# TorontoDeepLearning/convnet

Measured on NVIDIA H100. Metric: images/sec ImageNet AlexNet training, higher is better.
Workload: dtype bf16

## Files before the change

### convnet_b200/csrc/conv_tc.cu

```cuda
#include <cuda.h>
#include <cuda_bf16.h>
#include <cudaTypedefs.h>

#include <algorithm>
#include <vector>

#include "conv_kernels.h"
#include "sm90_ptx.cuh"

namespace cnb {

namespace {

constexpr int kConsumerWarps = 8;
template <int SW> constexpr int kThreadsFor = 32 * (kConsumerWarps + 1 + SW);
constexpr int BM = 128;
constexpr int BN_MAX = 128;
constexpr int BK = 32;
constexpr int kMaxStages = 8;
constexpr uint32_t kAStageBytes = BM * 128;
constexpr uint32_t kBStageBytes = BN_MAX * 128;

enum Op { kFprop = 0, kDgrad = 1, kWgrad = 2 };

struct TcParams {
  int bf16, chunk, chunk_shift, cpt, bk, nbc;
  int N, nb;
  int W, H, modX, modY, modules;
  int Cin, Cout;
  int kx, ky, sx, sy, px, py, taps;
  int frames, frame0;
  int BN, stages;
  int m_tiles, n_tiles, num_tiles;
  int kc_blocks;
  int x_mode, x_yblocks, x_ct;
  const float* xw;
  uint32_t bank_bytes;
  uint32_t epi_bytes;
  uint32_t b_tx_bytes;
  int a_merged, b_merged;
  int untied;
  int total_chunks;
  int splits, units_per_split;
  long long part_stride;
  float* out;
  __nv_bfloat16* out16;
  int vec;
  float st, so;
  const float* bias; int act;
  const float* mask; int mask_act;
  float drop_prob, drop_scale;
  unsigned long long drop_seed;
  long long out_frame_step;
  int o_sx, o_sy, o_x0, o_y0, o_W;
  long long out_plane;
};

struct __align__(8) SmemCtl {
  uint64_t full[kMaxStages];
  uint64_t empty[kMaxStages];
  uint64_t epi_full;
  uint64_t epi_empty;
};

struct Tile {
  int m_tile, n_tile;
  int tap, o_tile, c_tile, split;
};

template <int OP>
// ... 258 lines not shown
        const long long idx = row + col_stride * col;
        const float a[4] = {acc[k].x, acc[k].y, acc[k].z, acc[k].w};
        const float o[4] = {old[k].x, old[k].y, old[k].z, old[k].w};
        const float m[4] = {msk[k].x, msk[k].y, msk[k].z, msk[k].w};
        float v[4];
#pragma unroll
        for (int e = 0; e < 4; e++) {
          float r = so_eff * a[e];
          if (rmw) r += p.st * o[e];
          if (OP == kFprop) {
            if (bias) r += bv[k];
            if (SIG) { if (p.act) r = act_apply(r, p.act); }
            else if (p.act) r = fmaxf(r, 0.f);
            if (p.drop_scale != 0.f) r *= dropout_keep(p.drop_seed + (unsigned long long)(idx + e), p.drop_prob, p.drop_scale);
          }
          if (SIG) { if (p.mask) r = act_deriv(r, m[e], p.mask_act); }
          else if (p.mask && !(m[e] > 0.f)) r = 0.f;
          v[e] = r;
        }
        acc[k] = make_float4(v[0], v[1], v[2], v[3]);
      }
      if ((rmw || p.mask) && b + 1 < batches) load_batch(b + 1);
#pragma unroll
      for (int k = 0; k < kEpiCols; k++) {
        const int col = c0 + kStoreWarps * k;
        if (col >= ncols) continue;
        const long long idx = row + col_stride * col;
        const float v[4] = {acc[k].x, acc[k].y, acc[k].z, acc[k].w};
        float* const dst = p.out + idx;
        if (vec) {
          *reinterpret_cast<float4*>(dst) = acc[k];
        } else {
#pragma unroll
          for (int e = 0; e < 4; e++) dst[e] = v[e];
        }
        if (p.out16) {
          __nv_bfloat16* const d16 = p.out16 + idx;
          const __nv_bfloat162 lo = __floats2bfloat162_rn(v[0], v[1]), hi = __floats2bfloat162_rn(v[2], v[3]);
          if (vec) {
            uint2 w;
            w.x = *reinterpret_cast<const uint32_t*>(&lo);
            w.y = *reinterpret_cast<const uint32_t*>(&hi);
            *reinterpret_cast<uint2*>(d16) = w;
          } else {
            d16[0] = lo.x; d16[1] = lo.y; d16[2] = hi.x; d16[3] = hi.y;
          }
        }
      }
    }
    phase ^= 1;
  }
}

template <int OP, bool BF16, bool SIG, int SW>
__global__ void __launch_bounds__(kThreadsFor<SW>, 1)
tc_conv_kernel(const __grid_constant__ CUtensorMap mapA, const __grid_constant__ CUtensorMap mapB, const __grid_constant__ TcParams p) {
  extern __shared__ uint8_t smem_raw[];
  uint8_t* smem = reinterpret_cast<uint8_t*>((reinterpret_cast<uintptr_t>(smem_raw) + 1023) & ~uintptr_t(1023));
  uint8_t* smemA = smem;
  uint8_t* smemB = smem + (size_t)p.stages * kAStageBytes;
  uint8_t* smemE = smemB + (p.bank_bytes ? (size_t)p.bank_bytes : (size_t)p.stages * kBStageBytes);
  SmemCtl* ctl = reinterpret_cast<SmemCtl*>(smemE + p.epi_bytes);

  const int warp = __shfl_sync(0xffffffffu, (int)(threadIdx.x >> 5), 0), lane = threadIdx.x & 31;

  if (threadIdx.x == 0) {
    for (int s = 0; s < p.stages; s++) { ptx::mbar_init(&ctl->full[s], 1); ptx::mbar_init(&ctl->empty[s], kConsumerWarps); }
    ptx::mbar_init(&ctl->epi_full, kConsumerWarps);
    ptx::mbar_init(&ctl->epi_empty, SW);
    ptx::fence_barrier_init();
    ptx::tma_prefetch_desc(&mapA);
    ptx::tma_prefetch_desc(&mapB);
  }
  __syncthreads();
  ptx::pdl_launch_dependents();
  ptx::pdl_wait();

  if (warp > kConsumerWarps) {
    if constexpr (OP != kWgrad) store_tiles<OP, SIG, SW>(p, ctl, ptx::smem_u32(smemE), warp - kConsumerWarps - 1, lane);
    return;
  }
  if (warp == kConsumerWarps) {
    if (lane != 0) return;
    int stage = 0; uint32_t phase = 0;
    const uint32_t tx_bytes = kAStageBytes + p.b_tx_bytes;
    for (int t = blockIdx.x; t < p.num_tiles; t += gridDim.x) {
      const Tile tile = decode_tile<OP>(p, t);
      auto begin_stage = [&]() -> uint8_t* {
        ptx::mbar_wait(&ctl->empty[stage], phase ^ 1);
        ptx::mbar_arrive_expect_tx(&ctl->full[stage], tx_bytes);
        return smemA + (size_t)stage * kAStageBytes;
      };
      auto lda5 = [&](const void* m, void* dst, int c0, int c1, int c2, int c3, int c4) {
        ptx::tma_load_5d(m, &ctl->full[stage], dst, c0, c1, c2, c3, c4);
      };
      auto lda4 = [&](const void* m, void* dst, int c0, int c1, int c2, int c3) {
        ptx::tma_load_4d(m, &ctl->full[stage], dst, c0, c1, c2, c3);
      };
      auto lda3 = [&](const void* m, void* dst, int c0, int c1, int c2) {
        ptx::tma_load_3d(m, &ctl->full[stage], dst, c0, c1, c2);
      };
      auto end_stage = [&]() { if (++stage == p.stages) { stage = 0; phase ^= 1; } };

      if (OP == kFprop) {
        const Chunks ch = decode_chunks(p, tile.m_tile, p.modules);
        int cX[4], cY[4];
#pragma unroll
        for (int c = 0; c < 4; c++) {
          cX[c] = (ch.pos[c] % p.modX) * p.sx + p.px;
          cY[c] = (ch.pos[c] / p.modX) * p.sy + p.py;
        }
        if (p.x_mode) {
          for (int c = 0; c < p.Cin; c++)
            for (int yb = 0; yb < p.x_yblocks; yb++) {
              uint8_t* a = begin_stage();
              if (p.a_merged) {
                lda5(&mapA, a, 0, cX[0], cY[0] + 4 * yb, ch.n[0] >> 5, c);
              } else {
#pragma unroll
                for (int q = 0; q < 4; q++)
                  lda5(&mapA, a + q * (BK * 128), ch.n[q], c, cX[q], cY[q] + 4 * yb, ch.f[q]);
              }
              end_stage();
            }
        } else {
          const int cb0 = p.splits > 1 ? tile.split * p.units_per_split : 0;
          const int cb1 = p.splits > 1 ? min(cb0 + p.units_per_split, p.kc_blocks) : p.kc_blocks;
          const int mod = ch.pos[0];
          for (int ty = 0; ty < p.ky; ty++)
            for (int tx = 0; tx < p.kx; tx++) {
              const int tap = tx + p.kx * ty;
              for (int cb = cb0; cb < cb1; cb++) {
                uint8_t* a = begin_stage();
                uint8_t* b = smemB + (size_t)stage * kBStageBytes;
                if (p.a_merged) {
                  lda5(&mapA, a, 0, cb * p.bk, ch.n[0] >> p.chunk_shift, cX[0] + tx, cY[0] + ty);
                } else {
#pragma unroll
                  for (int c = 0; c < 4; c++)
                    if (c < p.cpt) lda5(&mapA, a + c * (p.bk * 128), ch.n[c], cb * p.bk, cX[c] + tx, cY[c] + ty, ch.f[c]);
                }
                const int o0 = tile.n_tile * p.BN;
                if (p.b_merged) {
                  if (p.untied) lda5(&mapB, b, 0, cb * p.bk, o0 >> p.chunk_shift, tap, mod);
                  else lda4(&mapB, b, 0, cb * p.bk, o0 >> p.chunk_shift, tap);
                } else {
                  for (int j = 0; j < ((p.BN + p.chunk - 1) >> p.chunk_shift); j++) {
                    if (p.untied) lda4(&mapB, b + j * (p.bk * 128), o0 + j * p.chunk, tap, cb * p.bk, mod);
                    else lda3(&mapB, b + j * (p.bk * 128), o0 + j * p.chunk, tap, cb * p.bk);
                  }
                }
                end_stage();
              }
            }
        }
      } else if (OP == kDgrad) {
        const Chunks ch = decode_chunks(p, tile.m_tile, p.W * p.H);
        const DgradTaps taps = dgrad_taps(p, ch);
        const bool none = dgrad_live_taps(p, taps) == 0;
        int cX[4], cY[4];
#pragma unroll
        for (int c = 0; c < 4; c++) { cX[c] = ch.pos[c] % p.W; cY[c] = ch.pos[c] / p.W; }
        const int ob0 = p.splits > 1 ? tile.split * p.units_per_split : 0;
        const int ob1 = p.splits > 1 ? min(ob0 + p.units_per_split, p.kc_blocks) : p.kc_blocks;
        for (int ty = 0; ty < p.ky; ty++)
          for (int tx = 0; tx < p.kx; tx++) {
            if (!(taps.any(tx, ty) || (none && tx == 0 && ty == 0))) continue;
            int mx[4], my[4];
#pragma unroll
            for (int c = 0; c < 4; c++) {
              const bool lv = ch.ok[c] && taps.live(c, tx, ty);
              mx[c] = lv ? (cX[c] - p.px - tx) / p.sx : -1;
              my[c] = lv ? (cY[c] - p.py - ty) / p.sy : -1;
            }
            const int tap = tx + p.kx * ty;
            const int mod = mx[0] >= 0 ? mx[0] + p.modX * my[0] : -1;
            for (int ob = ob0; ob < ob1; ob++) {
              uint8_t* a = begin_stage();
              uint8_t* b = smemB + (size_t)stage * kBStageBytes;
              if (p.a_merged) {
                lda5(&mapA, a, 0, ob * p.bk, ch.n[0] >> p.chunk_shift, mx[0], my[0]);
              } else {
#pragma unroll
                for (int c = 0; c < 4; c++)
                  if (c < p.cpt) lda5(&mapA, a + c * (p.bk * 128), ch.n[c], ob * p.bk, mx[c], my[c], p.frame0);
              }
              if (p.untied) lda4(&mapB, b, ob * p.bk, tap, tile.n_tile * p.BN, mod);
              else lda3(&mapB, b, ob * p.bk, tap, tile.n_tile * p.BN);
              end_stage();
            }
          }
      } else if (p.untied) {
        const int mx = tile.split % p.modX, my = tile.split / p.modX;
        const int X = mx * p.sx + p.px + tile.tap % p.kx, Y = my * p.sy + p.py + tile.tap / p.kx;
        for (int ib = 0; ib < p.nbc; ib++) {
          uint8_t* a = begin_stage();
          uint8_t* b = smemB + (size_t)stage * kBStageBytes;
          lda5(&mapA, a, ib * p.chunk, mx, my, tile.o_tile * BM, 0);
          lda5(&mapB, b, ib * p.chunk, X, Y, tile.c_tile * p.BN, 0);
          end_stage();
        }
      } else if (p.x_mode) {
        const int r0 = tile.split * p.units_per_split, r1 = min(r0 + p.units_per_split, p.modY * p.frames);
        const uint32_t c_bytes = (uint32_t)p.ky * 8 * 128;
        for (int r = r0; r < r1; r++) {
          const int f = r / p.modY, my = r % p.modY;
          for (int mx = 0; mx < p.modX; mx++)
            for (int ib = 0; ib < p.nb; ib++) {
              uint8_t* a = begin_stage();
              uint8_t* b = smemB + (size_t)stage * kBStageBytes;
              lda5(&mapA, a, ib * 32, mx, my, tile.o_tile * BM, f);
              for (int c = 0; c < p.x_ct; c++)
                lda5(&mapB, b + c * c_bytes, ib * 32, mx * p.sx + p.px, my * p.sy + p.py, tile.c_tile * p.x_ct + c, f);
              end_stage();
            }
        }
      } else {
        const WgradSpan sp = wgrad_span(p, tile);
        const int tx = tile.tap % p.kx, ty = tile.tap / p.kx;
        if (sp.live_rows == 0 || sp.mx_hi < sp.mx_lo) {
          for (int ib = 0; ib < p.nbc; ib++) {
            uint8_t* a = begin_stage();
            uint8_t* b = smemB + (size_t)stage * kBStageBytes;
            lda5(&mapA, a, ib * p.chunk, 0, 0, tile.o_tile * BM, 0);
            lda5(&mapB, b, ib * p.chunk, -1, -1, tile.c_tile * p.BN, 0);
            end_stage();
          }
        } else {
          for (int r = sp.r0; r < sp.r1; r++) {
            if (!wgrad_row_live(p, r, ty)) continue;
            const int f = r / p.modY, my = r % p.modY;
            const int Y = my * p.sy + p.py + ty;
            for (int mx = sp.mx_lo; mx <= sp.mx_hi; mx++) {
              const int X = mx * p.sx + p.px + tx;
              for (int ib = 0; ib < p.nbc; ib++) {
                uint8_t* a = begin_stage();
                uint8_t* b = smemB + (size_t)stage * kBStageBytes;
                lda5(&mapA, a, ib * p.chunk, mx, my, tile.o_tile * BM, f);
                lda5(&mapB, b, ib * p.chunk, X, Y, tile.c_tile * p.BN, f);
                end_stage();
              }
            }
          }
        }
      }
    }
    return;
  }

  const int g = lane >> 2, tq = lane & 3;
  const int row0 = warp * 16 + g;
  int stage = 0; uint32_t phase = 0;
  int bank_tile = -1;
  uint32_t epi_phase = 0;
  for (int t = blockIdx.x; t < p.num_tiles; t += gridDim.x) {
    const Tile tile = decode_tile<OP>(p, t);
    const int nkb = tile_kblocks<OP>(p, tile);
    float acc[BN_MAX / 8][4];
#pragma unroll
    for (int j = 0; j < BN_MAX / 8; j++)
#pragma unroll
      for (int e = 0; e < 4; e++) acc[j][e] = 0.f;

    if constexpr (BF16 || OP == kWgrad) {
      constexpr bool a_mn = (OP != kWgrad), b_mn = (OP == kFprop);
      constexpr uint32_t a_step = a_mn ? 2048u : 32u, b_step = b_mn ? 2048u : 32u;
      const uint64_t da0 = ptx::gmma_desc(ptx::smem_u32(smemA) + (uint32_t)(warp >> 2) * 8192u, a_mn ? 8192u : 16u, 1024u);
      const uint64_t db0 = ptx::gmma_desc(ptx::smem_u32(smemB), b_mn ? 8192u : 16u, 1024u);
      int prev = -1;
      ptx::wgmma_fence_operands(acc);
      for (int kb = 0; kb < nkb; kb++) {
        ptx::mbar_wait(&ctl->full[stage], phase);
        ptx::wgmma_fence();
        const uint64_t da = da0 + ((uint32_t)stage * kAStageBytes >> 4), db = db0 + ((uint32_t)stage * kBStageBytes >> 4);
#pragma unroll
        for (int ks = 0; ks < 4; ks++) {
          if constexpr (BF16)
            ptx::wgmma_m64n128k16_bf16<a_mn ? 1 : 0, b_mn ? 1 : 0>(acc, da + (ks * a_step >> 4), db + (ks * b_step >> 4));
          else
            ptx::wgmma_m64n128k8_tf32(acc, da + (ks * a_step >> 4), db + (ks * b_step >> 4));
        }
        ptx::wgmma_commit();
        ptx::wgmma_wait<1>();
        if (prev >= 0 && lane == 0) ptx::mbar_arrive(&ctl->empty[prev]);
        prev = stage;
        if (++stage == p.stages) { stage = 0; phase ^= 1; }
      }
      ptx::wgmma_wait<0>();
      ptx::wgmma_fence_operands(acc);
      if (prev >= 0 && lane == 0) ptx::mbar_arrive(&ctl->empty[prev]);
    } else if (OP == kFprop && p.x_mode) {
      if (tile.n_tile != bank_tile) {
        ptx::bar_sync(1, 32 * kConsumerWarps);
        xmode_fill_bank(p, smemB, tile.n_tile);
        ptx::fence_proxy_async_smem();
        ptx::bar_sync(1, 32 * kConsumerWarps);
        bank_tile = tile.n_tile;
      }
      const uint32_t sA = ptx::smem_u32(smemA), bank = ptx::smem_u32(smemB);
      switch (p.BN) {
        case 32: xmode_fprop_mma<32>(acc, p, ctl, sA, bank, nkb, stage, phase, row0, tq, lane); break;
        case 64: xmode_fprop_mma<64>(acc, p, ctl, sA, bank, nkb, stage, phase, row0, tq, lane); break;
        case 96: xmode_fprop_mma<96>(acc, p, ctl, sA, bank, nkb, stage, phase, row0, tq, lane); break;
        default: xmode_fprop_mma<128>(acc, p, ctl, sA, bank, nkb, stage, phase, row0, tq, lane); break;
      }
    } else {
      const uint32_t sA = ptx::smem_u32(smemA), sB = ptx::smem_u32(smemB);
      constexpr bool b_mn = (OP == kFprop);
      for (int kb = 0; kb < nkb; kb++) {
        ptx::mbar_wait(&ctl->full[stage], phase);
        const uint32_t A = sA + (uint32_t)stage * kAStageBytes, B = sB + (uint32_t)stage * kBStageBytes;
#pragma unroll
        for (int ks = 0; ks < 4; ks++) {
          const int k0 = ks * 8 + tq, k1 = k0 + 4;
          const uint32_t a0 = ptx::lds32(A + off_mnmajor(row0, k0));
          const uint32_t a1 = ptx::lds32(A + off_mnmajor(row0 + 8, k0));
          const uint32_t a2 = ptx::lds32(A + off_mnmajor(row0, k1));
          const uint32_t a3 = ptx::lds32(A + off_mnmajor(row0 + 8, k1));
#pragma unroll
          for (int j = 0; j < BN_MAX / 8; j++) {
            if (j * 8 >= p.BN) break;
            const int n = j * 8 + g;
            const uint32_t b0 = ptx::lds32(B + (b_mn ? off_mnmajor(n, k0) : off_kmajor(n, k0)));
            const uint32_t b1 = ptx::lds32(B + (b_mn ? off_mnmajor(n, k1) : off_kmajor(n, k1)));
            ptx::mma_tf32_16x8x8(acc[j], a0, a1, a2, a3, b0, b1);
          }
        }
        __syncwarp();
        if (lane == 0) ptx::mbar_arrive(&ctl->empty[stage]);
        if (++stage == p.stages) { stage = 0; phase ^= 1; }
      }
    }

    if constexpr (OP != kWgrad) {
      ptx::mbar_wait(&ctl->epi_empty, epi_phase ^ 1);
      uint32_t base[2][2];
#pragma unroll
      for (int h = 0; h < 2; h++)
#pragma unroll
        for (int e = 0; e < 2; e++) base[h][e] = ptx::smem_u32(smemE) + epi_off(row0 + 8 * h, 2 * tq + e);
#pragma unroll
      for (int j = 0; j < BN_MAX / 8; j++) {
        if (j * 8 >= p.BN) break;
#pragma unroll
        for (int h = 0; h < 2; h++)
#pragma unroll
          for (int e = 0; e < 2; e++) ptx::sts32(base[h][e] + j * 8 * BM * 4, acc[j][2 * h + e]);
      }
      __syncwarp();
      if (lane == 0) ptx::mbar_arrive(&ctl->epi_full);
      epi_phase ^= 1;
    } else {
      float* rowp[2] = {nullptr, nullptr};
      long long col_stride = 0;
#pragma unroll
      for (int h = 0; h < 2; h++) {
        const int o = tile.o_tile * BM + row0 + 8 * h;
        if (o < p.Cout) {
          rowp[h] = p.out + (long long)tile.split * p.Cout * p.taps * p.Cin + o;
          if (!p.x_mode) {
            col_stride = (long long)p.Cout * p.taps;
            rowp[h] += (long long)p.Cout * tile.tap + col_stride * ((long long)tile.c_tile * p.BN);
          }
        }
      }
      const int ncols_valid = p.x_mode ? min(p.BN, p.x_ct * p.ky * 8) : min(p.BN, p.Cin - tile.c_tile * p.BN);
      const bool direct_scale = (p.splits == 1) || p.untied;
      const float so_eff = direct_scale ? p.so : 1.f;
      const bool rmw = direct_scale && p.st != 0.f;
      auto dst_of = [&](float* rp, int col) -> float* {
        if (p.x_mode) {
          const int tx = col & 7, rr = col >> 3, ty = rr % p.ky, c = tile.c_tile * p.x_ct + rr / p.ky;
          if (tx >= p.kx || c >= p.Cin) return nullptr;
          return rp + (long long)p.Cout * (tx + p.kx * (ty + p.ky * c));
        }
        return rp + col_stride * col;
      };
#pragma unroll
      for (int h = 0; h < 2; h++) {
        float* const rp = rowp[h];
        if (rp == nullptr) continue;
#pragma unroll
        for (int j = 0; j < BN_MAX / 8; j++)
#pragma unroll
          for (int e = 0; e < 2; e++) {
            const int col = j * 8 + 2 * tq + e;
            if (col >= ncols_valid) continue;
            float* const dst = dst_of(rp, col);
            if (dst == nullptr) continue;
            float r = so_eff * acc[j][2 * h + e];
            if (rmw) r += p.st * *dst;
            *dst = r;
          }
      }
    }
  }
}

PFN_cuTensorMapEncodeTiled_v12000 encode_fn() {
  static PFN_cuTensorMapEncodeTiled_v12000 fn = nullptr;
  if (!fn) {
    void* ptr = nullptr;
    cudaDriverEntryPointQueryResult qres;
    CNB_CUDA_CHECK(cudaGetDriverEntryPoint("cuTensorMapEncodeTiled", &ptr, cudaEnableDefault, &qres));
    CNB_REQUIRE(qres == cudaDriverEntryPointSuccess && ptr != nullptr, "cuTensorMapEncodeTiled");
    fn = reinterpret_cast<PFN_cuTensorMapEncodeTiled_v12000>(ptr);
  }
  return fn;
}

struct Elem { int bf16, esz, chunk, shift, bk; };
inline Elem elem_for(bool bf16) { return bf16 ? Elem{1, 2, 64, 6, 64} : Elem{0, 4, 32, 5, 32}; }

bool make_map(CUtensorMap* map, const void* base, const Elem& e, int rank, const long long* dims, const long long* strides,
              const int* box) {
  cuuint64_t gdim[5], gstr[4];
  cuuint32_t bdim[5], estr[5];
  if ((reinterpret_cast<uintptr_t>(base) & 15) != 0) return false;
  for (int i = 0; i < rank; i++) {
    if (dims[i] <= 0 || dims[i] > 0xFFFFFFFFLL) return false;
    gdim[i] = (cuuint64_t)dims[i];
    bdim[i] = (cuuint32_t)box[i];
    estr[i] = 1;
    if (box[i] > 256) return false;
    if (i > 0) {
      const long long bytes = strides[i - 1] * e.esz;
      if (bytes % 16 != 0 || bytes <= 0 || bytes >= (1LL << 40)) return false;
      gstr[i - 1] = (cuuint64_t)bytes;
    }
  }
  CUresult r = encode_fn()(map, e.bf16 ? CU_TENSOR_MAP_DATA_TYPE_BFLOAT16 : CU_TENSOR_MAP_DATA_TYPE_FLOAT32, (cuuint32_t)rank,
                           const_cast<void*>(base), gdim, gstr, bdim, estr, CU_TENSOR_MAP_INTERLEAVE_NONE,
                           CU_TENSOR_MAP_SWIZZLE_128B, CU_TENSOR_MAP_L2_PROMOTION_L2_256B, CU_TENSOR_MAP_FLOAT_OOB_FILL_NONE);
  if (r != CUDA_SUCCESS) {
    fprintf(stderr, "convnet_b200: cuTensorMapEncodeTiled failed (%d)\n", (int)r);
    return false;
  }
  return true;
}

int pick_bn(int cols, int granule) {
  const int tiles = ceil_div(cols, BN_MAX);
  const int bn = ceil_div(ceil_div(cols, tiles), granule) * granule;
  return std::min(BN_MAX, std::max(granule, bn));
}

size_t smem_bytes_for(int stages, uint32_t bank_bytes, uint32_t epi_bytes) {
  const size_t b = bank_bytes ? (size_t)bank_bytes : (size_t)stages * kBStageBytes;
  return 1024 + (size_t)stages * kAStageBytes + b + epi_bytes + sizeof(SmemCtl) + 16;
}
constexpr size_t kSmemBudget = 227 * 1024;
inline uint32_t epi_bytes_for(int bn) { return (uint32_t)BM * bn * 4; }

int pick_stages(uint32_t bank_bytes, uint32_t epi_bytes) {
  int s = kMaxStages;
  while (s > 2 && smem_bytes_for(s, bank_bytes, epi_bytes) > kSmemBudget) s--;
  return s;
}

int pick_store_warps(int kblocks, double tile_bytes) {
  const double mma_us = 0.3 * kblocks;
  const double epi_us = tile_bytes / (3e6 / 132);
  return 2.0 * epi_us >= mma_us ? 7 : 3;
}

template <int OP, bool BF16, bool SIG, int SW>
void launch_one(const CUtensorMap& a, const CUtensorMap& b, const TcParams& p, size_t smem) {
  smem_opt_in(tc_conv_kernel<OP, BF16, SIG, SW>, 227 * 1024);
  const int grid = std::min(p.num_tiles, num_sms());
  launch_pdl(tc_conv_kernel<OP, BF16, SIG, SW>, dim3((unsigned)grid), dim3(kThreadsFor<SW>), smem, state().stream, a, b, p);
}

template <int OP>
void launch(const CUtensorMap& a, const CUtensorMap& b, TcParams& p) {
  p.epi_bytes = OP == kWgrad ? 0u : epi_bytes_for(p.BN);
  p.stages = pick_stages(p.bank_bytes, p.epi_bytes);
  const size_t smem = smem_bytes_for(p.stages, p.bank_bytes, p.epi_bytes);
  auto aligned = [](const void* q, uintptr_t a) { return (reinterpret_cast<uintptr_t>(q) & (a - 1)) == 0; };
  p.vec = aligned(p.out, 16) && aligned(p.mask, 16) && aligned(p.out16, 8) ? 1 : 0;
  const bool sig = p.act == kActLogistic || (p.mask && p.mask_act == kActLogistic);
  CNB_REQUIRE(OP != kWgrad || !sig, "tc_conv: wgrad has no activation epilogue");
  void (*run)(const CUtensorMap&, const CUtensorMap&, const TcParams&, size_t) = nullptr;
  if constexpr (OP != kWgrad) {
    const int kcb = p.splits > 1 ? p.units_per_split : p.kc_blocks;
    const int kblocks = (OP == kFprop && p.x_mode) ? p.Cin * p.x_yblocks : p.taps * kcb;
    const double bytes = BM * p.BN * (4.0 + (p.out16 ? 2 : 0) + (p.mask ? 4 : 0) + (p.st != 0.f && p.splits == 1 ? 4 : 0));
    if (pick_store_warps(kblocks, bytes) == 7) {
      if (sig) run = p.bf16 ? launch_one<OP, true, true, 7> : launch_one<OP, false, true, 7>;
      else run = p.bf16 ? launch_one<OP, true, false, 7> : launch_one<OP, false, false, 7>;
    } else if (sig) {
      run = p.bf16 ? launch_one<OP, true, true, 3> : launch_one<OP, false, true, 3>;
    }
  }
  if (!run) run = p.bf16 ? launch_one<OP, true, false, 3> : launch_one<OP, false, false, 3>;
  run(a, b, p, smem);
  count_launch();
  CNB_LAUNCH_CHECK("tc_conv");
}

void fill_common(TcParams& p, const ConvGeom& g, const Elem& e) {
  p.bf16 = e.bf16; p.chunk = e.chunk; p.chunk_shift = e.shift; p.cpt = BM / e.chunk; p.bk = e.bk;
  p.N = g.N; p.nb = ceil_div(g.N, 32); p.nbc = ceil_div(g.N, e.chunk);
  p.W = g.W; p.H = g.H; p.modX = g.modX; p.modY = g.modY; p.modules = g.modules;
  p.Cin = g.Cin; p.Cout = g.Cout;
  p.kx = g.kx; p.ky = g.ky; p.sx = g.sx; p.sy = g.sy; p.px = g.px; p.py = g.py; p.taps = g.kx * g.ky;
  p.frames = g.frames; p.frame0 = 0;
  p.splits = 1; p.units_per_split = 0; p.part_stride = 0;
  p.x_mode = 0; p.x_yblocks = 0; p.x_ct = 0; p.b_tx_bytes = 0;
  p.xw = nullptr; p.bank_bytes = 0; p.epi_bytes = 0;
  p.a_merged = 0; p.b_merged = 0;
  p.untied = g.conv ? 0 : 1;
  p.bias = nullptr; p.act = 0; p.mask = nullptr; p.mask_act = 0; p.out16 = nullptr; p.vec = 0;
  p.drop_prob = 0.f; p.drop_scale = 0.f; p.drop_seed = 0;
  p.o_sx = p.o_sy = 1; p.o_x0 = p.o_y0 = 0; p.o_W = g.modX; p.out_plane = g.modules;
  p.out_frame_step = g.out_frame_step;
  p.total_chunks = 0;
  p.st = 0.f; p.so = 1.f; p.out = nullptr;
}

bool image_map(CUtensorMap* m, const void* base, const Elem& e, const ConvGeom& g, int Wd, int Hd, int C,
               long long frame_step, bool channel_second, int box_c) {
  const long long N = g.N;
  if (channel_second) {
    const long long dims[5] = {N, C, Wd, Hd, g.frames};
    const long long str[4] = {N * Wd * Hd, N, N * Wd, frame_step};
    const int box[5] = {e.chunk, box_c, 1, 1, 1};
    return make_map(m, base, e, 5, dims, str, box);
  }
  const long long dims[5] = {N, Wd, Hd, C, g.frames};
  const long long str[4] = {N, N * Wd, N * Wd * Hd, frame_step};
  const int box[5] = {e.chunk, 1, 1, box_c, 1};
  return make_map(m, base, e, 5, dims, str, box);
}

bool merged_image_map(CUtensorMap* m, const void* base, const Elem& e, const ConvGeom& g, int Wd, int Hd, int C, bool x_mode) {
  const long long N = g.N;
  if (x_mode) {
    const long long dims[5] = {32, Wd, Hd, N / 32, C};
    const long long str[4] = {N, N * Wd, 32, N * Wd * Hd};
    const int box[5] = {32, 8, 4, 4, 1};
    return make_map(m, base, e, 5, dims, str, box);
  }
  const long long dims[5] = {e.chunk, C, N / e.chunk, Wd, Hd};
  const long long str[4] = {N * Wd * Hd, e.chunk, N, N * Wd};
  const int box[5] = {e.chunk, e.bk, BM / e.chunk, 1, 1};
// ... 239 lines not shown
  {
    const long long dims[4] = {g.Cout, (long long)g.kx * g.ky, g.Cin, g.modules};
    const long long str[3] = {g.Cout, (long long)g.Cout * g.kx * g.ky, (long long)g.Cout * g.K};
    const int box[4] = {e.chunk, 1, p.BN, 1};
    if (!make_map(&mb, buf.y, e, g.conv ? 3 : 4, dims, str, box)) return {};
  }
  float* out = targets + (long long)g.cin0 * g.H * g.W * g.N;
  bool emit = false;
  if (whole && p.splits > 1) {
    p.st = 0.f; p.out = buf.part; p.mask = nullptr;
    launch<kDgrad>(ma, mb, p);
    reduce_split(buf.part, out, out_elems, p.splits, st, so, nullptr, 1, 0, fuse.act_state, fuse.state_act);
  } else if (whole) {
    p.st = st; p.out = out; p.mask = fuse.act_state ? fuse.act_state + (long long)g.cin0 * g.H * g.W * g.N : nullptr;
    p.mask_act = fuse.state_act;
    p.out16 = out16;
    emit = out16 != nullptr;
    launch<kDgrad>(ma, mb, p);
  } else {
    scale_buffer(targets, g.img_total, st);
    p.st = 1.f;
    for (int f = 0; f < g.frames; f++) {
      p.frame0 = f; p.out = out + f * g.in_frame_step;
      launch<kDgrad>(ma, mb, p);
    }
  }
  return {bf ? kPathTcBf16 : kPathTcTf32, emit, false};
}
ConvOutcome tc_conv_down(const ConvGeom& g, const float* derivs, const float* filters, float* targets, float st, float so,
                         const Fuse& fuse, __nv_bfloat16* out16) {
  if (want_bf16()) {
    ConvOutcome r;
    if (st == 0.f) r = tc_conv_down_as_fprop(g, derivs, filters, targets, so, fuse, out16);
    if (r.path == kPathNone) r = tc_conv_down_impl(g, derivs, filters, targets, st, so, fuse, out16, true);
    if (r.path != kPathNone) return r;
  }
  return tc_conv_down_impl(g, derivs, filters, targets, st, so, fuse, out16, false);
}

static ConvPath tc_conv_outp_impl(const ConvGeom& g, const float* images, const float* derivs, float* targets, float st,
                                  float so, bool bf) {
  const Elem e = elem_for(bf);
  if (g.N % 4 != 0 || g.Cout < 8) return kPathNone;
  const bool x_mode = g.Cin < 8;
  if (x_mode && (g.kx > 8 || g.ky > 8)) return kPathNone;
  if (bf && (x_mode || g.N % 8 != 0 || !aligned16(images) || !aligned16(derivs))) return kPathNone;
  if (!g.conv && (g.N % 128 != 0 || g.frames != 1 || x_mode)) return kPathNone;
  if (bf && (long long)g.N * g.modules * g.frames < 1024 && !(g.frames == 1 && g.N % 128 == 0 && g.Cin % 32 == 0)) return kPathNone;
  TcParams p; fill_common(p, g, e);
  p.kc_blocks = 0;
  p.m_tiles = ceil_div(g.Cout, BM);
  if (x_mode) {
    p.x_mode = 1;
    p.x_ct = std::min(g.Cin, BN_MAX / (8 * g.ky));
    p.BN = ceil_div(p.x_ct * g.ky * 8, 16) * 16;
    p.n_tiles = ceil_div(g.Cin, p.x_ct);
    p.b_tx_bytes = (uint32_t)p.x_ct * g.ky * 8 * 128;
  } else {
    p.BN = pick_bn(g.Cin, 16);
    p.n_tiles = ceil_div(g.Cin, p.BN);
    p.b_tx_bytes = (uint32_t)p.BN * 128;
  }
  const int units = g.modY * g.frames;
  const long long base_tiles = (long long)(x_mode ? 1 : p.taps) * p.m_tiles * p.n_tiles;
  int splits;
  {
    const long long slots = num_sms();
    const double row_us = 0.3 * g.modX * std::max(1, p.nbc / 2);
    const double dw_bytes = 4.0 * g.Cout * g.K;
    const int cap = (int)std::max<long long>(1, std::min<long long>(units, (4LL * num_sms()) / std::max<long long>(base_tiles, 1)));
    double best = 1e30; splits = 1;
    for (int sp = 1; sp <= cap; sp++) {
      const int ups = ceil_div(units, sp), real = ceil_div(units, ups);
      const long long waves = ceil_div<long long>(base_tiles * real, slots);
      const double cost = (double)waves * (ups * row_us + 1.5) + (real > 1 ? dw_bytes * (real + 1) / 3e6 : 0.0);
      if (cost < best - 1e-9) { best = cost; splits = real; }
    }
  }
  const long long elems = (long long)g.Cout * g.K;
  while (splits > 1 && elems * splits * 4 > (1LL << 30)) splits--;
  p.units_per_split = ceil_div(units, splits);
  p.splits = ceil_div(units, p.units_per_split);
  if (!g.conv) {
    if (base_tiles * g.modules >= (1LL << 31)) return kPathNone;
    p.splits = g.modules; p.units_per_split = 1;
  }
  p.num_tiles = (int)(base_tiles * p.splits);
  p.st = st; p.so = so;
  CUtensorMap ma, mb;
  const bool partials = p.splits > 1 && g.conv;
  const size_t part_bytes = partials ? align_up(sizeof(float) * elems * p.splits) : 0;
  const CallBuffers buf = call_buffers(bf, part_bytes, {images, g.img_total, (long long)g.cin0 * g.H * g.W * g.N},
                                       {derivs, g.out_total, (long long)g.cout0 * g.modules * g.N});
  if (!image_map(&ma, buf.y, e, g, g.modX, g.modY, g.Cout, g.out_frame_step, false, BM)) return kPathNone;
  if (x_mode) {
    const long long N = g.N;
    const long long dims[5] = {N, g.W, g.H, g.Cin, g.frames};
    const long long str[4] = {N, N * g.W, N * g.W * g.H, g.in_frame_step};
    const int box[5] = {32, 8, g.ky, 1, 1};
    if (!make_map(&mb, buf.x, e, 5, dims, str, box)) return kPathNone;
  } else if (!image_map(&mb, buf.x, e, g, g.W, g.H, g.Cin, g.in_frame_step, false, p.BN)) return kPathNone;
  p.out = partials ? buf.part : targets;
  launch<kWgrad>(ma, mb, p);
  if (partials) reduce_partials(buf.part, targets, elems, 1, p.splits, st, so);
  return bf ? kPathTcBf16 : kPathTcTf32;
}
ConvPath tc_conv_outp(const ConvGeom& g, const float* images, const float* derivs, float* targets, float st, float so) {
  if (want_bf16()) {
    const ConvPath path = tc_conv_outp_impl(g, images, derivs, targets, st, so, true);
    if (path != kPathNone) return path;
  }
  return tc_conv_outp_impl(g, images, derivs, targets, st, so, false);
}

}
```

### convnet_b200/csrc/sm90_ptx.cuh

```cuda
#pragma once
#include <cuda_runtime.h>
#include <stdint.h>

namespace cnb {
namespace ptx {

__device__ __forceinline__ uint32_t smem_u32(const void* p) {
  return static_cast<uint32_t>(__cvta_generic_to_shared(p));
}

__device__ __forceinline__ void mbar_init(uint64_t* bar, uint32_t count) {
  asm volatile("mbarrier.init.shared::cta.b64 [%0], %1;" ::"r"(smem_u32(bar)), "r"(count));
}
__device__ __forceinline__ void fence_barrier_init() {
  asm volatile("fence.mbarrier_init.release.cluster;" ::: "memory");
}
__device__ __forceinline__ void mbar_arrive_expect_tx(uint64_t* bar, uint32_t bytes) {
  asm volatile("mbarrier.arrive.expect_tx.shared::cta.b64 _, [%0], %1;" ::"r"(smem_u32(bar)), "r"(bytes) : "memory");
}
__device__ __forceinline__ void mbar_arrive(uint64_t* bar) {
  asm volatile("mbarrier.arrive.shared::cta.b64 _, [%0];" ::"r"(smem_u32(bar)) : "memory");
}
__device__ __forceinline__ bool mbar_try_wait(uint64_t* bar, uint32_t parity) {
  uint32_t ok;
// ... 34 lines not shown
}
__device__ __forceinline__ void tma_load_3d(const void* desc, uint64_t* bar, void* dst, int c0, int c1, int c2) {
  asm volatile(
      "cp.async.bulk.tensor.3d.shared::cluster.global.mbarrier::complete_tx::bytes [%0], [%1, {%3, %4, %5}], [%2];"
      ::"r"(smem_u32(dst)), "l"(reinterpret_cast<uint64_t>(desc)), "r"(smem_u32(bar)), "r"(c0), "r"(c1), "r"(c2)
      : "memory");
}
__device__ __forceinline__ void tma_load_4d(const void* desc, uint64_t* bar, void* dst, int c0, int c1, int c2, int c3) {
  asm volatile(
      "cp.async.bulk.tensor.4d.shared::cluster.global.mbarrier::complete_tx::bytes [%0], [%1, {%3, %4, %5, %6}], [%2];"
      ::"r"(smem_u32(dst)), "l"(reinterpret_cast<uint64_t>(desc)), "r"(smem_u32(bar)), "r"(c0), "r"(c1), "r"(c2), "r"(c3)
      : "memory");
}
__device__ __forceinline__ void tma_load_5d(const void* desc, uint64_t* bar, void* dst, int c0, int c1, int c2, int c3,
                                            int c4) {
  asm volatile(
      "cp.async.bulk.tensor.5d.shared::cluster.global.mbarrier::complete_tx::bytes [%0], [%1, {%3, %4, %5, %6, %7}], [%2];"
      ::"r"(smem_u32(dst)), "l"(reinterpret_cast<uint64_t>(desc)), "r"(smem_u32(bar)), "r"(c0), "r"(c1), "r"(c2),
      "r"(c3), "r"(c4)
      : "memory");
}

__device__ __forceinline__ void pdl_wait() { asm volatile("griddepcontrol.wait;" ::: "memory"); }
__device__ __forceinline__ void pdl_launch_dependents() { asm volatile("griddepcontrol.launch_dependents;" ::: "memory"); }

__device__ __forceinline__ uint32_t lds32(uint32_t addr) {
  uint32_t v; asm volatile("ld.shared.b32 %0, [%1];" : "=r"(v) : "r"(addr) : "memory"); return v;
}
__device__ __forceinline__ float4 lds128(uint32_t addr) {
  float4 v;
  asm volatile("ld.shared.v4.f32 {%0, %1, %2, %3}, [%4];" : "=f"(v.x), "=f"(v.y), "=f"(v.z), "=f"(v.w) : "r"(addr) : "memory");
  return v;
}
__device__ __forceinline__ void sts32(uint32_t addr, float v) {
  asm volatile("st.shared.f32 [%0], %1;" ::"r"(addr), "f"(v) : "memory");
}

__device__ __forceinline__ void mma_tf32_16x8x8(float (&d)[4], uint32_t a0, uint32_t a1, uint32_t a2, uint32_t a3,
                                                uint32_t b0, uint32_t b1) {
  asm volatile("mma.sync.aligned.m16n8k8.row.col.f32.tf32.tf32.f32 {%0, %1, %2, %3}, {%4, %5, %6, %7}, {%8, %9}, "
               "{%0, %1, %2, %3};"
               : "+f"(d[0]), "+f"(d[1]), "+f"(d[2]), "+f"(d[3])
               : "r"(a0), "r"(a1), "r"(a2), "r"(a3), "r"(b0), "r"(b1));
}

__device__ __forceinline__ uint64_t gmma_desc(uint32_t smem_addr, uint32_t lbo_bytes, uint32_t sbo_bytes) {
  return (uint64_t)((smem_addr >> 4) & 0x3FFF) | ((uint64_t)((lbo_bytes >> 4) & 0x3FFF) << 16) |
         ((uint64_t)((sbo_bytes >> 4) & 0x3FFF) << 32) | (1ULL << 62);
}
__device__ __forceinline__ void wgmma_fence() { asm volatile("wgmma.fence.sync.aligned;" ::: "memory"); }
__device__ __forceinline__ void wgmma_commit() { asm volatile("wgmma.commit_group.sync.aligned;" ::: "memory"); }
template <int N>
__device__ __forceinline__ void wgmma_wait() { asm volatile("wgmma.wait_group.sync.aligned %0;" ::"n"(N) : "memory"); }
__device__ __forceinline__ void wgmma_fence_operands(float (&d)[16][4]) {
#pragma unroll
  for (int j = 0; j < 16; j++)
#pragma unroll
    for (int e = 0; e < 4; e++) asm volatile("" : "+f"(d[j][e])::"memory");
}

#define CNB_ACC4(j) "+f"(d[j][0]), "+f"(d[j][1]), "+f"(d[j][2]), "+f"(d[j][3])
template <int TA, int TB>
__device__ __forceinline__ void wgmma_m64n128k16_bf16(float (&d)[16][4], uint64_t desc_a, uint64_t desc_b) {
  asm volatile(
      "{\n\t.reg .pred p;\n\tsetp.ne.b32 p, %68, 0;\n\t"
      "wgmma.mma_async.sync.aligned.m64n128k16.f32.bf16.bf16 "
      "{%0, %1, %2, %3, %4, %5, %6, %7, %8, %9, %10, %11, %12, %13, %14, %15, "
      "%16, %17, %18, %19, %20, %21, %22, %23, %24, %25, %26, %27, %28, %29, %30, %31, "
      "%32, %33, %34, %35, %36, %37, %38, %39, %40, %41, %42, %43, %44, %45, %46, %47, "
      "%48, %49, %50, %51, %52, %53, %54, %55, %56, %57, %58, %59, %60, %61, %62, %63}, "
      "%64, %65, p, 1, 1, %66, %67;\n\t}"
      : CNB_ACC4(0), CNB_ACC4(1), CNB_ACC4(2), CNB_ACC4(3), CNB_ACC4(4), CNB_ACC4(5), CNB_ACC4(6), CNB_ACC4(7),
        CNB_ACC4(8), CNB_ACC4(9), CNB_ACC4(10), CNB_ACC4(11), CNB_ACC4(12), CNB_ACC4(13), CNB_ACC4(14), CNB_ACC4(15)
      : "l"(desc_a), "l"(desc_b), "n"(TA), "n"(TB), "r"(1));
}

__device__ __forceinline__ void wgmma_m64n128k8_tf32(float (&d)[16][4], uint64_t desc_a, uint64_t desc_b) {
  asm volatile(
      "{\n\t.reg .pred p;\n\tsetp.ne.b32 p, %66, 0;\n\t"
      "wgmma.mma_async.sync.aligned.m64n128k8.f32.tf32.tf32 "
      "{%0, %1, %2, %3, %4, %5, %6, %7, %8, %9, %10, %11, %12, %13, %14, %15, "
      "%16, %17, %18, %19, %20, %21, %22, %23, %24, %25, %26, %27, %28, %29, %30, %31, "
      "%32, %33, %34, %35, %36, %37, %38, %39, %40, %41, %42, %43, %44, %45, %46, %47, "
      "%48, %49, %50, %51, %52, %53, %54, %55, %56, %57, %58, %59, %60, %61, %62, %63}, "
      "%64, %65, p, 1, 1;\n\t}"
      : CNB_ACC4(0), CNB_ACC4(1), CNB_ACC4(2), CNB_ACC4(3), CNB_ACC4(4), CNB_ACC4(5), CNB_ACC4(6), CNB_ACC4(7),
        CNB_ACC4(8), CNB_ACC4(9), CNB_ACC4(10), CNB_ACC4(11), CNB_ACC4(12), CNB_ACC4(13), CNB_ACC4(14), CNB_ACC4(15)
      : "l"(desc_a), "l"(desc_b), "r"(1));
}

template <int N>
__device__ __forceinline__ void wgmma_m64nNk8_tf32_rs(float (&d)[16][4], const uint32_t (&a)[4], uint64_t desc_b) {
  static_assert(N == 32 || N == 64 || N == 96 || N == 128, "tf32 RS wgmma: N in {32, 64, 96, 128}");
  if constexpr (N == 32) {
    asm volatile(
        "{\n\t.reg .pred p;\n\tsetp.ne.b32 p, %21, 0;\n\t"
        "wgmma.mma_async.sync.aligned.m64n32k8.f32.tf32.tf32 "
        "{%0, %1, %2, %3, %4, %5, %6, %7, %8, %9, %10, %11, %12, %13, %14, %15}, "
        "{%16, %17, %18, %19}, %20, p, 1, 1;\n\t}"
        : CNB_ACC4(0), CNB_ACC4(1), CNB_ACC4(2), CNB_ACC4(3)
        : "r"(a[0]), "r"(a[1]), "r"(a[2]), "r"(a[3]), "l"(desc_b), "r"(1));
  } else if constexpr (N == 64) {
    asm volatile(
        "{\n\t.reg .pred p;\n\tsetp.ne.b32 p, %37, 0;\n\t"
        "wgmma.mma_async.sync.aligned.m64n64k8.f32.tf32.tf32 "
        "{%0, %1, %2, %3, %4, %5, %6, %7, %8, %9, %10, %11, %12, %13, %14, %15, "
        "%16, %17, %18, %19, %20, %21, %22, %23, %24, %25, %26, %27, %28, %29, %30, %31}, "
        "{%32, %33, %34, %35}, %36, p, 1, 1;\n\t}"
        : CNB_ACC4(0), CNB_ACC4(1), CNB_ACC4(2), CNB_ACC4(3), CNB_ACC4(4), CNB_ACC4(5), CNB_ACC4(6), CNB_ACC4(7)
        : "r"(a[0]), "r"(a[1]), "r"(a[2]), "r"(a[3]), "l"(desc_b), "r"(1));
  } else if constexpr (N == 96) {
    asm volatile(
        "{\n\t.reg .pred p;\n\tsetp.ne.b32 p, %53, 0;\n\t"
        "wgmma.mma_async.sync.aligned.m64n96k8.f32.tf32.tf32 "
        "{%0, %1, %2, %3, %4, %5, %6, %7, %8, %9, %10, %11, %12, %13, %14, %15, "
        "%16, %17, %18, %19, %20, %21, %22, %23, %24, %25, %26, %27, %28, %29, %30, %31, "
        "%32, %33, %34, %35, %36, %37, %38, %39, %40, %41, %42, %43, %44, %45, %46, %47}, "
        "{%48, %49, %50, %51}, %52, p, 1, 1;\n\t}"
        : CNB_ACC4(0), CNB_ACC4(1), CNB_ACC4(2), CNB_ACC4(3), CNB_ACC4(4), CNB_ACC4(5), CNB_ACC4(6), CNB_ACC4(7),
          CNB_ACC4(8), CNB_ACC4(9), CNB_ACC4(10), CNB_ACC4(11)
        : "r"(a[0]), "r"(a[1]), "r"(a[2]), "r"(a[3]), "l"(desc_b), "r"(1));
  } else {
    asm volatile(
        "{\n\t.reg .pred p;\n\tsetp.ne.b32 p, %69, 0;\n\t"
        "wgmma.mma_async.sync.aligned.m64n128k8.f32.tf32.tf32 "
        "{%0, %1, %2, %3, %4, %5, %6, %7, %8, %9, %10, %11, %12, %13, %14, %15, "
        "%16, %17, %18, %19, %20, %21, %22, %23, %24, %25, %26, %27, %28, %29, %30, %31, "
        "%32, %33, %34, %35, %36, %37, %38, %39, %40, %41, %42, %43, %44, %45, %46, %47, "
        "%48, %49, %50, %51, %52, %53, %54, %55, %56, %57, %58, %59, %60, %61, %62, %63}, "
        "{%64, %65, %66, %67}, %68, p, 1, 1;\n\t}"
        : CNB_ACC4(0), CNB_ACC4(1), CNB_ACC4(2), CNB_ACC4(3), CNB_ACC4(4), CNB_ACC4(5), CNB_ACC4(6), CNB_ACC4(7),
          CNB_ACC4(8), CNB_ACC4(9), CNB_ACC4(10), CNB_ACC4(11), CNB_ACC4(12), CNB_ACC4(13), CNB_ACC4(14), CNB_ACC4(15)
        : "r"(a[0]), "r"(a[1]), "r"(a[2]), "r"(a[3]), "l"(desc_b), "r"(1));
  }
}
#undef CNB_ACC4

__device__ __forceinline__ void fence_proxy_async_smem() { asm volatile("fence.proxy.async.shared::cta;" ::: "memory"); }
__device__ __forceinline__ void bar_sync(int id, int threads) {
  asm volatile("bar.sync %0, %1;" ::"r"(id), "r"(threads) : "memory");
}

}
// ... 2 lines not shown
```

Before: 16200.

## Add wide 168-column tf32 wgrad tile for x_mode weight gradients

```diff
diff --git a/convnet_b200/csrc/conv_tc.cu b/convnet_b200/csrc/conv_tc.cu
--- a/convnet_b200/csrc/conv_tc.cu
+++ b/convnet_b200/csrc/conv_tc.cu
@@ -16,6 +16,7 @@
 template <int SW> constexpr int kThreadsFor = 32 * (kConsumerWarps + 1 + SW);
 constexpr int BM = 128;
 constexpr int BN_MAX = 128;
+constexpr int kWideN = 168;
 constexpr int BK = 32;
 constexpr int kMaxStages = 8;
 constexpr uint32_t kAStageBytes = BM * 128;
@@ -380,14 +381,16 @@
   }
 }
 
-template <int OP, bool BF16, bool SIG, int SW>
+template <int OP, bool BF16, bool SIG, int SW, int ACC_N = BN_MAX>
 __global__ void __launch_bounds__(kThreadsFor<SW>, 1)
 tc_conv_kernel(const __grid_constant__ CUtensorMap mapA, const __grid_constant__ CUtensorMap mapB, const __grid_constant__ TcParams p) {
+  static_assert(ACC_N == BN_MAX || (ACC_N == kWideN && OP == kWgrad && !BF16), "the wide tile is tf32 wgrad only");
+  constexpr uint32_t kBStage = (uint32_t)ACC_N * 128;
   extern __shared__ uint8_t smem_raw[];
   uint8_t* smem = reinterpret_cast<uint8_t*>((reinterpret_cast<uintptr_t>(smem_raw) + 1023) & ~uintptr_t(1023));
   uint8_t* smemA = smem;
   uint8_t* smemB = smem + (size_t)p.stages * kAStageBytes;
-  uint8_t* smemE = smemB + (p.bank_bytes ? (size_t)p.bank_bytes : (size_t)p.stages * kBStageBytes);
+  uint8_t* smemE = smemB + (p.bank_bytes ? (size_t)p.bank_bytes : (size_t)p.stages * kBStage);
   SmemCtl* ctl = reinterpret_cast<SmemCtl*>(smemE + p.epi_bytes);
 
   const int warp = __shfl_sync(0xffffffffu, (int)(threadIdx.x >> 5), 0), lane = threadIdx.x & 31;
@@ -460,7 +463,7 @@
               const int tap = tx + p.kx * ty;
               for (int cb = cb0; cb < cb1; cb++) {
                 uint8_t* a = begin_stage();
-                uint8_t* b = smemB + (size_t)stage * kBStageBytes;
+                uint8_t* b = smemB + (size_t)stage * kBStage;
                 if (p.a_merged) {
                   lda5(&mapA, a, 0, cb * p.bk, ch.n[0] >> p.chunk_shift, cX[0] + tx, cY[0] + ty);
                 } else {
@@ -505,7 +508,7 @@
             const int mod = mx[0] >= 0 ? mx[0] + p.modX * my[0] : -1;
             for (int ob = ob0; ob < ob1; ob++) {
               uint8_t* a = begin_stage();
-              uint8_t* b = smemB + (size_t)stage * kBStageBytes;
+              uint8_t* b = smemB + (size_t)stage * kBStage;
               if (p.a_merged) {
                 lda5(&mapA, a, 0, ob * p.bk, ch.n[0] >> p.chunk_shift, mx[0], my[0]);
               } else {
@@ -523,7 +526,7 @@
         const int X = mx * p.sx + p.px + tile.tap % p.kx, Y = my * p.sy + p.py + tile.tap / p.kx;
         for (int ib = 0; ib < p.nbc; ib++) {
           uint8_t* a = begin_stage();
-          uint8_t* b = smemB + (size_t)stage * kBStageBytes;
+          uint8_t* b = smemB + (size_t)stage * kBStage;
           lda5(&mapA, a, ib * p.chunk, mx, my, tile.o_tile * BM, 0);
           lda5(&mapB, b, ib * p.chunk, X, Y, tile.c_tile * p.BN, 0);
           end_stage();
@@ -536,7 +539,7 @@
           for (int mx = 0; mx < p.modX; mx++)
             for (int ib = 0; ib < p.nb; ib++) {
               uint8_t* a = begin_stage();
-              uint8_t* b = smemB + (size_t)stage * kBStageBytes;
+              uint8_t* b = smemB + (size_t)stage * kBStage;
               lda5(&mapA, a, ib * 32, mx, my, tile.o_tile * BM, f);
               for (int c = 0; c < p.x_ct; c++)
                 lda5(&mapB, b + c * c_bytes, ib * 32, mx * p.sx + p.px, my * p.sy + p.py, tile.c_tile * p.x_ct + c, f);
@@ -549,7 +552,7 @@
         if (sp.live_rows == 0 || sp.mx_hi < sp.mx_lo) {
           for (int ib = 0; ib < p.nbc; ib++) {
             uint8_t* a = begin_stage();
-            uint8_t* b = smemB + (size_t)stage * kBStageBytes;
+            uint8_t* b = smemB + (size_t)stage * kBStage;
             lda5(&mapA, a, ib * p.chunk, 0, 0, tile.o_tile * BM, 0);
             lda5(&mapB, b, ib * p.chunk, -1, -1, tile.c_tile * p.BN, 0);
             end_stage();
@@ -563,7 +566,7 @@
               const int X = mx * p.sx + p.px + tx;
               for (int ib = 0; ib < p.nbc; ib++) {
                 uint8_t* a = begin_stage();
-                uint8_t* b = smemB + (size_t)stage * kBStageBytes;
+                uint8_t* b = smemB + (size_t)stage * kBStage;
                 lda5(&mapA, a, ib * p.chunk, mx, my, tile.o_tile * BM, f);
                 lda5(&mapB, b, ib * p.chunk, X, Y, tile.c_tile * p.BN, f);
                 end_stage();
@@ -584,9 +587,9 @@
   for (int t = blockIdx.x; t < p.num_tiles; t += gridDim.x) {
     const Tile tile = decode_tile<OP>(p, t);
     const int nkb = tile_kblocks<OP>(p, tile);
-    float acc[BN_MAX / 8][4];
-#pragma unroll
-    for (int j = 0; j < BN_MAX / 8; j++)
+    float acc[ACC_N / 8][4];
+#pragma unroll
+    for (int j = 0; j < ACC_N / 8; j++)
 #pragma unroll
       for (int e = 0; e < 4; e++) acc[j][e] = 0.f;
 
@@ -600,11 +603,13 @@
       for (int kb = 0; kb < nkb; kb++) {
         ptx::mbar_wait(&ctl->full[stage], phase);
         ptx::wgmma_fence();
-        const uint64_t da = da0 + ((uint32_t)stage * kAStageBytes >> 4), db = db0 + ((uint32_t)stage * kBStageBytes >> 4);
+        const uint64_t da = da0 + ((uint32_t)stage * kAStageBytes >> 4), db = db0 + ((uint32_t)stage * kBStage >> 4);
 #pragma unroll
         for (int ks = 0; ks < 4; ks++) {
           if constexpr (BF16)
             ptx::wgmma_m64n128k16_bf16<a_mn ? 1 : 0, b_mn ? 1 : 0>(acc, da + (ks * a_step >> 4), db + (ks * b_step >> 4));
+          else if constexpr (ACC_N == kWideN)
+            ptx::wgmma_m64n168k8_tf32(acc, da + (ks * a_step >> 4), db + (ks * b_step >> 4));
           else
             ptx::wgmma_m64n128k8_tf32(acc, da + (ks * a_step >> 4), db + (ks * b_step >> 4));
         }
@@ -637,7 +642,7 @@
       constexpr bool b_mn = (OP == kFprop);
       for (int kb = 0; kb < nkb; kb++) {
         ptx::mbar_wait(&ctl->full[stage], phase);
-        const uint32_t A = sA + (uint32_t)stage * kAStageBytes, B = sB + (uint32_t)stage * kBStageBytes;
+        const uint32_t A = sA + (uint32_t)stage * kAStageBytes, B = sB + (uint32_t)stage * kBStage;
 #pragma unroll
         for (int ks = 0; ks < 4; ks++) {
           const int k0 = ks * 8 + tq, k1 = k0 + 4;
@@ -709,7 +714,7 @@
         float* const rp = rowp[h];
         if (rp == nullptr) continue;
 #pragma unroll
-        for (int j = 0; j < BN_MAX / 8; j++)
+        for (int j = 0; j < ACC_N / 8; j++)
 #pragma unroll
           for (int e = 0; e < 2; e++) {
             const int col = j * 8 + 2 * tq + e;
@@ -773,16 +778,16 @@
   return std::min(BN_MAX, std::max(granule, bn));
 }
 
-size_t smem_bytes_for(int stages, uint32_t bank_bytes, uint32_t epi_bytes) {
-  const size_t b = bank_bytes ? (size_t)bank_bytes : (size_t)stages * kBStageBytes;
+size_t smem_bytes_for(int stages, uint32_t bank_bytes, uint32_t epi_bytes, uint32_t b_stage = kBStageBytes) {
+  const size_t b = bank_bytes ? (size_t)bank_bytes : (size_t)stages * b_stage;
   return 1024 + (size_t)stages * kAStageBytes + b + epi_bytes + sizeof(SmemCtl) + 16;
 }
 constexpr size_t kSmemBudget = 227 * 1024;
 inline uint32_t epi_bytes_for(int bn) { return (uint32_t)BM * bn * 4; }
 
-int pick_stages(uint32_t bank_bytes, uint32_t epi_bytes) {
+int pick_stages(uint32_t bank_bytes, uint32_t epi_bytes, uint32_t b_stage) {
   int s = kMaxStages;
-  while (s > 2 && smem_bytes_for(s, bank_bytes, epi_bytes) > kSmemBudget) s--;
+  while (s > 2 && smem_bytes_for(s, bank_bytes, epi_bytes, b_stage) > kSmemBudget) s--;
   return s;
 }
 
@@ -792,18 +797,22 @@
   return 2.0 * epi_us >= mma_us ? 7 : 3;
 }
 
-template <int OP, bool BF16, bool SIG, int SW>
+template <int OP, bool BF16, bool SIG, int SW, int ACC_N = BN_MAX>
 void launch_one(const CUtensorMap& a, const CUtensorMap& b, const TcParams& p, size_t smem) {
-  smem_opt_in(tc_conv_kernel<OP, BF16, SIG, SW>, 227 * 1024);
+  smem_opt_in(tc_conv_kernel<OP, BF16, SIG, SW, ACC_N>, 227 * 1024);
   const int grid = std::min(p.num_tiles, num_sms());
-  launch_pdl(tc_conv_kernel<OP, BF16, SIG, SW>, dim3((unsigned)grid), dim3(kThreadsFor<SW>), smem, state().stream, a, b, p);
+  launch_pdl(tc_conv_kernel<OP, BF16, SIG, SW, ACC_N>, dim3((unsigned)grid), dim3(kThreadsFor<SW>), smem, state().stream, a,
+             b, p);
 }
 
 template <int OP>
 void launch(const CUtensorMap& a, const CUtensorMap& b, TcParams& p) {
+  const bool wide = OP == kWgrad && p.BN > BN_MAX;
+  CNB_REQUIRE(!wide || (p.x_mode && !p.bf16 && p.x_ct * p.ky * 8 <= kWideN), "tc_conv: wide wgrad tile");
   p.epi_bytes = OP == kWgrad ? 0u : epi_bytes_for(p.BN);
-  p.stages = pick_stages(p.bank_bytes, p.epi_bytes);
-  const size_t smem = smem_bytes_for(p.stages, p.bank_bytes, p.epi_bytes);
+  const uint32_t b_stage = wide ? (uint32_t)kWideN * 128 : kBStageBytes;
+  p.stages = pick_stages(p.bank_bytes, p.epi_bytes, b_stage);
+  const size_t smem = smem_bytes_for(p.stages, p.bank_bytes, p.epi_bytes, b_stage);
   auto aligned = [](const void* q, uintptr_t a) { return (reinterpret_cast<uintptr_t>(q) & (a - 1)) == 0; };
   p.vec = aligned(p.out, 16) && aligned(p.mask, 16) && aligned(p.out16, 8) ? 1 : 0;
   const bool sig = p.act == kActLogistic || (p.mask && p.mask_act == kActLogistic);
@@ -819,6 +828,9 @@
     } else if (sig) {
       run = p.bf16 ? launch_one<OP, true, true, 3> : launch_one<OP, false, true, 3>;
     }
+  }
+  if constexpr (OP == kWgrad) {
+    if (wide) run = launch_one<OP, false, false, 3, kWideN>;
   }
   if (!run) run = p.bf16 ? launch_one<OP, true, false, 3> : launch_one<OP, false, false, 3>;
   run(a, b, p, smem);
@@ -1164,8 +1176,8 @@
   p.m_tiles = ceil_div(g.Cout, BM);
   if (x_mode) {
     p.x_mode = 1;
-    p.x_ct = std::min(g.Cin, BN_MAX / (8 * g.ky));
-    p.BN = ceil_div(p.x_ct * g.ky * 8, 16) * 16;
+    p.x_ct = std::min(g.Cin, kWideN / (8 * g.ky));
+    p.BN = p.x_ct * g.ky * 8;
     p.n_tiles = ceil_div(g.Cin, p.x_ct);
     p.b_tx_bytes = (uint32_t)p.x_ct * g.ky * 8 * 128;
   } else {
@@ -1175,16 +1187,18 @@
   }
   const int units = g.modY * g.frames;
   const long long base_tiles = (long long)(x_mode ? 1 : p.taps) * p.m_tiles * p.n_tiles;
+  const long long split_tiles =
+      x_mode ? (long long)p.m_tiles * ceil_div(g.Cin, std::min(g.Cin, BN_MAX / (8 * g.ky))) : base_tiles;
   int splits;
   {
     const long long slots = num_sms();
     const double row_us = 0.3 * g.modX * std::max(1, p.nbc / 2);
     const double dw_bytes = 4.0 * g.Cout * g.K;
-    const int cap = (int)std::max<long long>(1, std::min<long long>(units, (4LL * num_sms()) / std::max<long long>(base_tiles, 1)));
+    const int cap = (int)std::max<long long>(1, std::min<long long>(units, (4LL * num_sms()) / std::max<long long>(split_tiles, 1)));
     double best = 1e30; splits = 1;
     for (int sp = 1; sp <= cap; sp++) {
       const int ups = ceil_div(units, sp), real = ceil_div(units, ups);
-      const long long waves = ceil_div<long long>(base_tiles * real, slots);
+      const long long waves = ceil_div<long long>(split_tiles * real, slots);
       const double cost = (double)waves * (ups * row_us + 1.5) + (real > 1 ? dw_bytes * (real + 1) / 3e6 : 0.0);
       if (cost < best - 1e-9) { best = cost; splits = real; }
     }
diff --git a/convnet_b200/csrc/sm90_ptx.cuh b/convnet_b200/csrc/sm90_ptx.cuh
--- a/convnet_b200/csrc/sm90_ptx.cuh
+++ b/convnet_b200/csrc/sm90_ptx.cuh
@@ -110,9 +110,10 @@
 __device__ __forceinline__ void wgmma_commit() { asm volatile("wgmma.commit_group.sync.aligned;" ::: "memory"); }
 template <int N>
 __device__ __forceinline__ void wgmma_wait() { asm volatile("wgmma.wait_group.sync.aligned %0;" ::"n"(N) : "memory"); }
-__device__ __forceinline__ void wgmma_fence_operands(float (&d)[16][4]) {
+template <int J>
+__device__ __forceinline__ void wgmma_fence_operands(float (&d)[J][4]) {
 #pragma unroll
-  for (int j = 0; j < 16; j++)
+  for (int j = 0; j < J; j++)
 #pragma unroll
     for (int e = 0; e < 4; e++) asm volatile("" : "+f"(d[j][e])::"memory");
 }
@@ -147,6 +148,23 @@
       : "l"(desc_a), "l"(desc_b), "r"(1));
 }
 
+__device__ __forceinline__ void wgmma_m64n168k8_tf32(float (&d)[21][4], uint64_t desc_a, uint64_t desc_b) {
+  asm volatile(
+      "{\n\t.reg .pred p;\n\tsetp.ne.b32 p, %86, 0;\n\t"
+      "wgmma.mma_async.sync.aligned.m64n168k8.f32.tf32.tf32 "
+      "{%0, %1, %2, %3, %4, %5, %6, %7, %8, %9, %10, %11, %12, %13, %14, %15, "
+      "%16, %17, %18, %19, %20, %21, %22, %23, %24, %25, %26, %27, %28, %29, %30, %31, "
+      "%32, %33, %34, %35, %36, %37, %38, %39, %40, %41, %42, %43, %44, %45, %46, %47, "
+      "%48, %49, %50, %51, %52, %53, %54, %55, %56, %57, %58, %59, %60, %61, %62, %63, "
+      "%64, %65, %66, %67, %68, %69, %70, %71, %72, %73, %74, %75, %76, %77, %78, %79, "
+      "%80, %81, %82, %83}, "
+      "%84, %85, p, 1, 1;\n\t}"
+      : CNB_ACC4(0), CNB_ACC4(1), CNB_ACC4(2), CNB_ACC4(3), CNB_ACC4(4), CNB_ACC4(5), CNB_ACC4(6), CNB_ACC4(7),
+        CNB_ACC4(8), CNB_ACC4(9), CNB_ACC4(10), CNB_ACC4(11), CNB_ACC4(12), CNB_ACC4(13), CNB_ACC4(14), CNB_ACC4(15),
+        CNB_ACC4(16), CNB_ACC4(17), CNB_ACC4(18), CNB_ACC4(19), CNB_ACC4(20)
+      : "l"(desc_a), "l"(desc_b), "r"(1));
+}
+
 template <int N>
 __device__ __forceinline__ void wgmma_m64nNk8_tf32_rs(float (&d)[16][4], const uint32_t (&a)[4], uint64_t desc_b) {
   static_assert(N == 32 || N == 64 || N == 96 || N == 128, "tf32 RS wgmma: N in {32, 64, 96, 128}");
```

Result: faster. 16370 (median of 6 runs) (+1.1%).
